# uber-research/deep-neuroevolution

Hardware: NVIDIA H100
Metric: env-steps/sec across ES population (whole box) (higher is better)
Workload: dtype f32

## Files before the change

### deep-neuroevolution_b200/csrc/common.cuh

```cuda
#pragma once
#include <cuda_runtime.h>
#include <stdint.h>
#include <stdio.h>
#include <stdarg.h>
#include <string.h>

#include "../../include/dne.h"

#if defined(__CUDA_ARCH__) && (__CUDA_ARCH__ != 900)
#error "libdne is written for sm_90a (H100) only"
#endif

#define DNE_MAX_PREP 16
struct dne_ctx {
    int device;
    int sm_count;
    const float* noise;
    int64_t noise_count;
    double* scratch;
    cudaEvent_t* ev;
    int ev_cap, ev_n, prof_on;
    void* ev_wait;
    void* ev_record;
    int ev_record_done;
    int ev_mode;
    struct { const void* ws; const float* theta; int n_slots; } prep[DNE_MAX_PREP];
};
void dne_prep_invalidate_theta(dne_ctx* ctx, const float* d_theta);
extern unsigned long long g_dne_launches;
#define DNE_LAUNCHED(n) (g_dne_launches += (unsigned long long)(n))
#define DNE_SCRATCH_DOUBLES 16384

void dne_set_error(const char* fmt, ...);

#define DNE_CHECK_ARG(cond, msg)                                   \
    do {                                                           \
        if (!(cond)) {                                             \
            dne_set_error("%s: %s", __func__, msg);                \
            return DNE_ERR_ARG;                                    \
        }                                                          \
    } while (0)

#define DNE_CUDA(call)                                                                 \
    do {                                                                               \
        cudaError_t e__ = (call);                                                      \
        if (e__ != cudaSuccess) {                                                      \
            dne_set_error("%s: %s -> %s", __func__, #call, cudaGetErrorString(e__));   \
            return DNE_ERR_CUDA;                                                       \
        }                                                                              \
    } while (0)

#define DNE_LAUNCH_CHECK1() do { DNE_LAUNCHED(1); DNE_LAUNCH_CHECK(); } while (0)
// ... 83 lines not shown
```

### deep-neuroevolution_b200/csrc/dne_api.cu

```cuda
#include "common.cuh"
#include "forward.cuh"

static thread_local char g_err[512] = "";
unsigned long long g_dne_launches = 0;
int g_dne_theta_tma = 1;
int g_dne_chain_ticks = 0;
int g_dne_pdl = 1;
int g_dne_fold_theta = 1;
int g_dne_fuse_head = 1;

void dne_set_error(const char* fmt, ...) {
    va_list ap;
    va_start(ap, fmt);
    vsnprintf(g_err, sizeof(g_err), fmt, ap);
    va_end(ap);
}

extern "C" const char* dne_last_error(void) { return g_err; }
extern "C" int dne_version(void) { return 100; }
extern "C" int dne_abi_sizes(int* layer_desc_bytes, int* net_desc_bytes) {
    if (layer_desc_bytes) *layer_desc_bytes = (int)sizeof(dne_layer_desc);
    if (net_desc_bytes) *net_desc_bytes = (int)sizeof(dne_net_desc);
    return DNE_OK;
}

extern "C" int dne_ctx_create(int device, dne_ctx** out) {
    DNE_CHECK_ARG(out, "out is null");
    *out = nullptr;
    int n = 0;
    DNE_CUDA(cudaGetDeviceCount(&n));
    DNE_CHECK_ARG(device >= 0 && device < n, "no such CUDA device");
    DNE_CUDA(cudaSetDevice(device));
    cudaDeviceProp prop;
    DNE_CUDA(cudaGetDeviceProperties(&prop, device));
    if (prop.major != 9 || prop.minor != 0) {
        dne_set_error("dne_ctx_create: device %d is sm_%d%d; libdne is built for sm_90a (H100) only", device,
                      prop.major, prop.minor);
        return DNE_ERR_CUDA;
    }
    dne_ctx* c = new dne_ctx();
    c->device = device;
    c->sm_count = prop.multiProcessorCount;
    c->noise = nullptr;
    c->noise_count = 0;
    c->scratch = nullptr;
    c->ev = nullptr;
    c->ev_cap = c->ev_n = c->prof_on = 0;
    c->ev_wait = c->ev_record = nullptr;
    c->ev_record_done = 0;
    c->ev_mode = 0;
    for (int i = 0; i < DNE_MAX_PREP; ++i) c->prep[i].ws = nullptr, c->prep[i].theta = nullptr;
    cudaError_t e = cudaMalloc(&c->scratch, sizeof(double) * DNE_SCRATCH_DOUBLES);
    if (e != cudaSuccess) {
        delete c;
        dne_set_error("dne_ctx_create: cudaMalloc -> %s", cudaGetErrorString(e));
        return DNE_ERR_CUDA;
    }
    *out = c;
    return DNE_OK;
}

extern "C" int dne_ctx_destroy(dne_ctx* ctx) {
    if (!ctx) return DNE_OK;
    cudaSetDevice(ctx->device);
    if (ctx->scratch) cudaFree(ctx->scratch);
    if (ctx->ev) {
        for (int i = 0; i < 2 * ctx->ev_cap; ++i) cudaEventDestroy(ctx->ev[i]);
        delete[] ctx->ev;
    }
    delete ctx;
    return DNE_OK;
}

extern "C" int dne_set_option(const char* name, int value) {
    DNE_CHECK_ARG(name, "name is null");
    if (strcmp(name, "conv_tc") == 0 && value >= 0 && value <= 2) { g_dne_conv_tc = value; return DNE_OK; }
    if (strcmp(name, "gemv_bulk") == 0) { g_dne_gemv_bulk = value ? 1 : 0; return DNE_OK; }
    if (strcmp(name, "fuse_head") == 0) { g_dne_fuse_head = value ? 1 : 0; return DNE_OK; }
    if (strcmp(name, "theta_mc") == 0) { extern int g_dne_theta_mc; g_dne_theta_mc = value ? 1 : 0; return DNE_OK; }
    if (strcmp(name, "theta_tma") == 0) { g_dne_theta_tma = value ? 1 : 0; return DNE_OK; }
    if (strcmp(name, "gemv_stages") == 0 && value >= 2 && value <= 8) { extern int g_dne_gemv_stages; g_dne_gemv_stages = value; return DNE_OK; }
    if (strcmp(name, "fold_theta") == 0 && value >= 0 && value <= 1) { g_dne_fold_theta = value; return DNE_OK; }
    if (strcmp(name, "chain_ticks") == 0 && value >= 0 && value <= 1) { g_dne_chain_ticks = value; return DNE_OK; }
    if (strcmp(name, "pdl") == 0 && value >= 0 && value <= 1) { g_dne_pdl = value; return DNE_OK; }
    if (strcmp(name, "gemv_grid") == 0 && value >= 0) { extern int g_dne_gemv_grid; g_dne_gemv_grid = value; return DNE_OK; }
    if (strcmp(name, "gemv_ctas_per_sm") == 0 && value >= 1 && value <= 2) { g_dne_gemv_ctas_per_sm = value; return DNE_OK; }
    dne_set_error("dne_set_option: unknown option '%s'", name);
    return DNE_ERR_ARG;
}

extern "C" long long dne_launch_count(int reset) {
    const long long v = (long long)g_dne_launches;
    if (reset) g_dne_launches = 0;
    return v;
}

extern "C" int dne_profile_enable(dne_ctx* ctx, int on, int capacity) {
    DNE_CHECK_ARG(ctx, "ctx is null");
    if (on == 2) {
        ctx->prof_on = ctx->ev ? 1 : 0;
        return DNE_OK;
    }
    if (on) {
        if (capacity < 1) capacity = 4096;
        if (capacity > ctx->ev_cap) {
            if (ctx->ev) {
                for (int i = 0; i < 2 * ctx->ev_cap; ++i) cudaEventDestroy(ctx->ev[i]);
                delete[] ctx->ev;
            }
            ctx->ev = new cudaEvent_t[2 * (size_t)capacity];
            for (int i = 0; i < 2 * capacity; ++i) DNE_CUDA(cudaEventCreate(&ctx->ev[i]));
            ctx->ev_cap = capacity;
        }
        ctx->ev_n = 0;
    }
    ctx->prof_on = on ? 1 : 0;
    return DNE_OK;
}

extern "C" int dne_profile_read(dne_ctx* ctx, int* n_launches, double* total_ms) {
    DNE_CHECK_ARG(ctx && n_launches && total_ms, "bad arguments");
    DNE_CUDA(cudaDeviceSynchronize());
    double tot = 0.0;
    for (int i = 0; i < ctx->ev_n; ++i) {
        float ms = 0.f;
        DNE_CUDA(cudaEventElapsedTime(&ms, ctx->ev[2 * i], ctx->ev[2 * i + 1]));
        tot += ms;
    }
    *n_launches = ctx->ev_n;
    *total_ms = tot;
    return DNE_OK;
}

extern "C" int dne_noise_bind(dne_ctx* ctx, const float* d_noise, int64_t count) {
    DNE_CHECK_ARG(ctx && d_noise && count > 0, "bad arguments");
    DNE_CHECK_ARG(((uintptr_t)d_noise & 15) == 0, "noise table must be 16-byte aligned");
    ctx->noise = d_noise;
    ctx->noise_count = count;
    return DNE_OK;
}

constexpr int PLAN_SM_COUNT = 132;

struct ForwardPlan {
    size_t x0_off;
    size_t act_off[DNE_MAX_LAYERS];
    int64_t act_elems[DNE_MAX_LAYERS];
    DensePlan dense[DNE_MAX_LAYERS];
    size_t part_theta_off, part_noise_off;
    size_t xc_off[DNE_MAX_LAYERS], wc_off[DNE_MAX_LAYERS];
    size_t total;
};

static bool tgm_candidate(const dne_net_desc* net, int l, const DensePlan& dp) {
    if (l == 0 || net->layers[l].kind != DNE_DENSE || net->layers[l - 1].kind != DNE_CONV || !dp.decomposed) return false;
    if (!dne_s2d_supported(net->layers[l - 1], l - 1 == 0)) return false;
    return dne_tgm_supported(net->layers[l].cin, net->layers[l].cout, dp.k_per_split);
}

static int64_t layer_out_elems(const dne_layer_desc& L) {
    return L.kind == DNE_CONV ? (int64_t)L.hout * L.hout * L.cout : (int64_t)L.cout;
}

static int plan_forward(const dne_net_desc* net, int n_slots, int paired, bool shared_theta, ForwardPlan* fp) {
// ... 370 lines not shown
```

### deep-neuroevolution_b200/csrc/forward.cuh

```cuda
#pragma once
#include "common.cuh"

struct SlotArgs {
    const float* theta;
    const float* noise;
    const int64_t* noise_idx;
    const float* scale;
    const int32_t* theta_idx;
    const uint8_t* active;
    int64_t P;
};

struct LayerEpi {
    int64_t off_b, off_beta, off_gamma;
    int act, bn, bn_off, vbn_len;
    const float* vbn;
};

struct GemvSrc {
    const float* base;
    const int64_t* idx64;
    const int32_t* idx32;
    int64_t mul, off;
};

extern int g_dne_gemv_bulk;
extern int g_dne_fold_theta;
extern int g_dne_gemv_ctas_per_sm;
int dne_launch_member_gemm_tc(const SlotArgs& sa, int64_t off_w, int64_t off_b, const float* X, int64_t x_slot_stride, int M,
                              int K, int N, float* out, int64_t out_slot_stride, int n_slots, cudaStream_t st);
constexpr int DNE_GEMV_BLOCK_ROWS = 256;
int dne_gemv_pieces(int K);
int dne_launch_gemv_union(const SlotArgs& sa, const GemvSrc& src, int G, const float* X, int64_t x_slot_stride, int K,
                          int N, int n_pieces, int n_slots, float* part, int sm_count, cudaStream_t st,
                          const float* fold_theta = nullptr, int fold_n_split = 0);

struct DensePlan {
    bool decomposed;
    int n_split, k_per_split;
    int G, Gt, rows_per_chunk, n_chunks, rw;
    size_t part_theta_floats, part_noise_floats;
};

extern int g_dne_conv_tc;
int dne_launch_conv_layer_tc(const SlotArgs& sa, const dne_layer_desc& L, const LayerEpi& epi, bool in_u8,
                             const void* in, int64_t in_slot_stride, int64_t in_img_stride, float* out,
                             int64_t out_slot_stride, int64_t out_img_stride, int n_slots, int n_img,
                             cudaStream_t st);
int dne_launch_conv_layer_simt(const SlotArgs& sa, const dne_layer_desc& L, const LayerEpi& epi, bool in_u8,
                               const void* in, int64_t in_slot_stride, int64_t in_img_stride, float* out,
                               int64_t out_slot_stride, int64_t out_img_stride, int n_slots, int n_img,
                               cudaStream_t st);

DensePlan dne_plan_dense(const dne_layer_desc& L, int n_slots, int paired, bool shared_theta, int sm_count);

int dne_launch_conv_layer(const SlotArgs& sa, const dne_layer_desc& L, const LayerEpi& epi, bool in_u8,
                          const void* in, int64_t in_slot_stride, int64_t in_img_stride, float* out,
                          int64_t out_slot_stride, int64_t out_img_stride, int n_slots, int n_img,
                          cudaStream_t st);

struct DenseHead {
    const dne_layer_desc* L;
    LayerEpi epi;
    float* out;
    int64_t out_slot_stride;
    int32_t* actions;
};
bool dne_head_fusable(const dne_layer_desc& L, const DensePlan& p, const dne_layer_desc& head, const DensePlan& hp);
// ... 41 lines not shown
```

### deep-neuroevolution_b200/csrc/forward_kernels.cu

```cuda
#include "common.cuh"
#include "forward.cuh"
#include "epilogue.cuh"

constexpr int CONV_BK = 16;

template <int CIN, int COUT, int KS, int STRIDE, int HIN, int HOUT, int PAD, bool IN_U8, int BM, int TM, int TN>
__global__ void __launch_bounds__((BM / TM) * (COUT / TN))
conv_kernel(SlotArgs sa, int64_t off_w, LayerEpi epi, const void* __restrict__ in_base, int64_t in_slot_stride,
            int64_t in_img_stride, float* __restrict__ out_base, int64_t out_slot_stride, int64_t out_img_stride) {
    constexpr int THREADS = (BM / TM) * (COUT / TN);
    constexpr int M = HOUT * HOUT;
    constexpr int K = KS * KS * CIN;
    constexpr int BK = CONV_BK;
    static_assert(K % BK == 0 && CIN % 4 == 0 && TM % 4 == 0, "tile constraints");
    constexpr int A_UNITS = BM * BK / 4;
    constexpr int A_PER_THREAD = (A_UNITS + THREADS - 1) / THREADS;
    constexpr int B_ELEMS = BK * COUT;
    constexpr int B_PER_THREAD = (B_ELEMS + THREADS - 1) / THREADS;

    const int slot = blockIdx.y;
    if (!slot_active(sa, slot)) return;
    const int img = blockIdx.z;
    const int m_tile = blockIdx.x * BM;
    const int tid = threadIdx.x;
// ... 591 lines not shown
}

int dne_launch_dense_layer(const dne_ctx* ctx, const SlotArgs& sa, const dne_layer_desc& L, const LayerEpi& epi,
                           const DensePlan& p, const float* X, int64_t x_slot_stride, float* out,
                           int64_t out_slot_stride, int32_t* actions, float* part_theta, float* part_noise,
                           int n_slots, cudaStream_t st, const DenseHead* head, const TgmOperands* tgm) {
    const int K = L.cin, N = L.cout;
    if (!p.decomposed) {
        if (actions && N > DS_MAXN) return DNE_ERR_UNSUP;
        dense_small_kernel<<<dim3(n_slots, (N + DS_MAXN - 1) / DS_MAXN), DS_THREADS, 0, st>>>(
            sa, L.off_w, epi, X, x_slot_stride, K, N, out, out_slot_stride, actions);
        DNE_LAUNCHED(1);
        return 0;
    }
    if (x_slot_stride != K || actions) return DNE_ERR_UNSUP;
    const int threads = (N / 4) * p.rw;
    auto gemv_smem = [&](int G) {
        size_t sm1 = (size_t)G * (p.rows_per_chunk + 1) * sizeof(float);
        size_t sm2 = (size_t)p.rw * G * (N + 4) * sizeof(float);
        return sm1 > sm2 ? sm1 : sm2;
    };
    if (p.Gt == 0) {
        if (tgm && dne_launch_theta_gemm_tma(tgm->Xc, tgm->Wc, n_slots, K, N, p.k_per_split, p.n_split, part_theta, st) == 0) {
        } else if (!(g_dne_conv_tc && dne_launch_theta_gemm_tc(X, n_slots, K, N, sa.theta + L.off_w, p.k_per_split, p.n_split,
                                                        part_theta, st) == 0)) {
            dim3 grid((N + DG_BN - 1) / DG_BN, (n_slots + DG_BM - 1) / DG_BM, p.n_split);
            dense_theta_gemm_kernel<<<grid, DG_THREADS, 0, st>>>(X, n_slots, K, N, sa.theta + L.off_w, p.k_per_split,
                                                                part_theta);
        }
    } else {
        GemvSrc ts{sa.theta, nullptr, sa.theta_idx, sa.P, L.off_w};
        dim3 grid(p.n_chunks, (n_slots + p.Gt - 1) / p.Gt);
        if (g_dne_gemv_bulk && dne_launch_gemv_union(sa, ts, p.Gt, X, x_slot_stride, K, N, p.n_chunks, n_slots, part_theta,
                                                     ctx->sm_count, st) == 0) {
        } else if (p.Gt == 2)
            dense_noise_gemv_kernel<2, 8><<<grid, threads, gemv_smem(2), st>>>(sa, ts, X, x_slot_stride, K, N,
                                                                              p.rows_per_chunk, part_theta);
        else
            dense_noise_gemv_kernel<1, 8><<<grid, threads, gemv_smem(1), st>>>(sa, ts, X, x_slot_stride, K, N,
                                                                              p.rows_per_chunk, part_theta);
    }
    bool folded = false;
    {
        GemvSrc ns{sa.noise, sa.noise_idx, nullptr, 0, L.off_w};
        dne_ctx* mctx = const_cast<dne_ctx*>(ctx);
        const bool first_gemv = !ctx->ev_record_done;
        if (first_gemv && ctx->ev_mode == 0 && ctx->ev_record) {
            cudaEventRecord((cudaEvent_t)ctx->ev_record, st);
            mctx->ev_record_done = 1;
        }
        if (first_gemv && ctx->ev_mode == 1 && ctx->ev_wait) {
            cudaStreamWaitEvent(st, (cudaEvent_t)ctx->ev_wait, 0);
            mctx->ev_wait = nullptr;
        }
        const int groups = (n_slots + p.G - 1) / p.G;
        dim3 grid(p.n_chunks, groups);
        const bool prof = ctx->prof_on && ctx->ev_n < ctx->ev_cap;
        if (prof) cudaEventRecord(ctx->ev[2 * ctx->ev_n], st);
        folded = g_dne_gemv_bulk && g_dne_fold_theta && p.Gt == 0;
        if (g_dne_gemv_bulk && dne_launch_gemv_union(sa, ns, p.G, X, x_slot_stride, K, N, p.n_chunks, n_slots, part_noise,
                                                     ctx->sm_count, st, folded ? part_theta : nullptr,
                                                     folded ? p.n_split : 0) == 0) {
        } else if ((folded = false), p.G == 2)
            dense_noise_gemv_kernel<2, 8><<<grid, threads, gemv_smem(2), st>>>(sa, ns, X, x_slot_stride, K, N,
                                                                              p.rows_per_chunk, part_noise);
        else
            dense_noise_gemv_kernel<1, 8><<<grid, threads, gemv_smem(1), st>>>(sa, ns, X, x_slot_stride, K, N,
                                                                              p.rows_per_chunk, part_noise);
        if (prof) {
            cudaEventRecord(ctx->ev[2 * ctx->ev_n + 1], st);
            const_cast<dne_ctx*>(ctx)->ev_n++;
        }
        if (first_gemv && ctx->ev_mode == 1 && ctx->ev_record) {
            cudaEventRecord((cudaEvent_t)ctx->ev_record, st);
            mctx->ev_record_done = 1;
        }
    }
    if (head) {
        if (dne_launch_chain(dense_combine_head_kernel, dim3(n_slots), dim3(DCH_THREADS), 0, st, true, sa, epi, n_slots, N, p.G,
                             (const float*)part_theta, folded ? -1 : p.n_split, p.Gt, (const float*)part_noise, p.n_chunks, out, out_slot_stride,
                             (int64_t)head->L->off_w, head->epi, (int)head->L->cout, head->out, head->out_slot_stride,
                             head->actions) != cudaSuccess)
            return DNE_ERR_CUDA;
    } else {
        dim3 grid((N + 255) / 256, n_slots);
        dense_combine_kernel<<<grid, 256, 0, st>>>(sa, epi, n_slots, N, p.G, part_theta, folded ? -1 : p.n_split, p.Gt, part_noise,
                                                  p.n_chunks, out, out_slot_stride);
    }
    DNE_LAUNCHED(3);
    return 0;
}

void dne_launch_ob_norm(const float* obs, const float* mean, const float* stdv, int64_t total, int dim, float* out,
                        cudaStream_t st) {
// ... 4 lines not shown
```

### deep-neuroevolution_b200/csrc/gemv_bulk.cu

```cuda
#include <climits>
#include "common.cuh"
#include "forward.cuh"
#include "epilogue.cuh"
#include "wgmma.cuh"

using namespace wg;

int g_dne_gemv_bulk = 1;
int g_dne_gemv_ctas_per_sm = 2;
int g_dne_gemv_grid = 0;
int g_dne_gemv_stages = 5;

constexpr int GB_CONSUMERS = 256;
constexpr int GB_THREADS = GB_CONSUMERS + 32;
constexpr int GB_STAGES = 8;
constexpr int GB_STAGE_BYTES = 16384;
constexpr int GB_RPR = 4;
constexpr int GU_BLK = DNE_GEMV_BLOCK_ROWS;
constexpr int GU_VEC = 8;
constexpr int GU_VB = 4;
constexpr int GU_MIN_N = 64;
constexpr int GU_XS_LD_MAX = GU_BLK + 4096 / GU_MIN_N;
constexpr int GU_XS_FLOATS = GU_VEC * GU_XS_LD_MAX > (1024 / GU_MIN_N) * GU_VB * (GU_MIN_N + 4)
                                 ? GU_VEC * GU_XS_LD_MAX : (1024 / GU_MIN_N) * GU_VB * (GU_MIN_N + 4);
constexpr int GU_PLAN_BYTES_PER_GROUP = 8 + 5 * 4;

__device__ __forceinline__ int gu_cover(const int* pb0, const int* pb1, int n_groups, int b, int first, int cap, int* out,
                                        int lane) {
    int total = 0;
    for (int h0 = 0; h0 < n_groups; h0 += 32) {
        const int h = h0 + lane;
        const bool c = h < n_groups && pb0[h] <= b && b <= pb1[h];
        const unsigned m = __ballot_sync(0xffffffffu, c);
        const int ord = total + __popc(m & ((1u << lane) - 1u));
        if (c && ord >= first && ord < first + cap) out[ord - first] = h;
        total += __popc(m);
    }
    __syncwarp();
    return total;
}

template <int G>
__global__ void __launch_bounds__(GB_THREADS, 2)
gemv_union_kernel(SlotArgs sa, GemvSrc src, const float* __restrict__ X, int64_t x_slot_stride, int K, int N,
                  int n_pieces, int n_groups, int n_slots, float* __restrict__ part, int n_stages,
                  const float* __restrict__ tpart, int t_split) {
    constexpr int CAP = GU_VEC / G;
    extern __shared__ uint8_t smem_raw[];
    uint8_t* smem = (uint8_t*)(((uintptr_t)smem_raw + 127) & ~(uintptr_t)127);
    float* stage_base = reinterpret_cast<float*>(smem);
    int64_t* pE0 = reinterpret_cast<int64_t*>(smem + n_stages * GB_STAGE_BYTES);
    int* pb0 = reinterpret_cast<int*>(pE0 + n_groups);
    int* pb1 = pb0 + n_groups;
    int* psort = pb1 + n_groups;
    int* pstart = psort + n_groups;
    int* ppre = pstart + n_groups;
    __shared__ uint64_t full_bar[GB_STAGES], empty_bar[GB_STAGES];
    __shared__ __align__(16) float xs[GU_XS_FLOATS];
    __shared__ int cov_c[CAP], cov_p[CAP];
    __shared__ int rho_c[CAP];
    __shared__ int s_total, s_row0, s_nelem, s_items;

    const int tid = threadIdx.x, warp = tid >> 5, lane = tid & 31;
    const int NQ = N >> 2;
    const int RW = GB_CONSUMERS / NQ;
    const int RB = GB_RPR * RW;
    const int XS_LD = GU_BLK + RB;
    pdl_trigger();

    if (tid == 0) {
        for (int s = 0; s < n_stages; ++s) {
            mbar_init(&full_bar[s], 1);
            mbar_init(&empty_bar[s], GB_CONSUMERS / 32);
        }
        fence_mbar_init();
    }
    for (int g = tid; g < n_groups; g += GB_THREADS) {
        const int slot0 = g * G;
        bool any = false;
#pragma unroll
        for (int m = 0; m < G; ++m) any = any || (slot0 + m < n_slots && slot_active(sa, slot0 + m));
        const int64_t E0 = (src.idx64 ? src.idx64[slot0] : (src.idx32 ? (int64_t)src.idx32[slot0] * src.mul : 0)) + src.off;
        pE0[g] = E0;
        pb0[g] = any ? (int)(E0 / N / GU_BLK) : INT_MAX;
        pb1[g] = any ? (int)((E0 + (int64_t)K * N - 1) / N / GU_BLK) : -1;
    }
    __syncthreads();
    for (int g = tid; g < n_groups; g += GB_THREADS) {
        const int key = pb0[g];
        int r = 0;
        for (int h = 0; h < n_groups; ++h) {
            const int kh = pb0[h];
            r += (kh < key) || (kh == key && h < g);
        }
        psort[r] = g;
    }
    __syncthreads();
    if (warp == 0) {
        int carry_max = -1, carry_sum = 0;
        for (int i0 = 0; i0 < n_groups; i0 += 32) {
            const int i = i0 + lane;
            const int g = i < n_groups ? psort[i] : 0;
            const int b0 = i < n_groups ? pb0[g] : INT_MAX, b1 = i < n_groups ? pb1[g] : -1;
            int mx = b1;
#pragma unroll
            for (int d = 1; d < 32; d <<= 1) {
                const int o = __shfl_up_sync(0xffffffffu, mx, d);
                if (lane >= d) mx = max(mx, o);
            }
            int before = __shfl_up_sync(0xffffffffu, mx, 1);
            if (lane == 0) before = -1;
            before = max(before, carry_max);
            const int start = max(b0, before + 1);
            const int add = (b0 != INT_MAX && b1 >= start) ? b1 - start + 1 : 0;
            int sum = add;
#pragma unroll
            for (int d = 1; d < 32; d <<= 1) {
                const int o = __shfl_up_sync(0xffffffffu, sum, d);
                if (lane >= d) sum += o;
            }
            if (i < n_groups) { pstart[i] = start; ppre[i] = carry_sum + sum - add; }
            carry_sum += __shfl_sync(0xffffffffu, sum, 31);
            carry_max = max(carry_max, __shfl_sync(0xffffffffu, mx, 31));
        }
        if (lane == 0) s_items = carry_sum;
    }
    __syncthreads();
    const int n_items = s_items;
    auto item_block = [&](int q) {
        int lo = 0, hi = n_groups;
        while (lo < hi) {
            const int mid = (lo + hi) >> 1;
            if (ppre[mid] <= q) lo = mid + 1; else hi = mid;
        }
        return pstart[lo - 1] + (q - ppre[lo - 1]);
    };
    auto pass_range = [&](int b, const int* gl, int ng, int64_t& row0, int& n_elem) {
        int64_t r_first = INT64_MAX, e_last = 0;
        for (int i = 0; i < ng; ++i) {
            const int64_t E0 = pE0[gl[i]];
            r_first = min(r_first, E0 / N);
            e_last = max(e_last, (E0 + (int64_t)K * N + 3) & ~(int64_t)3);
        }
        const int64_t blk0 = (int64_t)b * GU_BLK;
        row0 = max(r_first, blk0);
        const int64_t e_end = min(e_last, (blk0 + GU_BLK) * N);
        n_elem = (int)(e_end - row0 * N);
    };

    if (warp == GB_CONSUMERS / 32) {
        uint32_t it = 0;
        for (int item = blockIdx.x; item < n_items; item += gridDim.x) {
            const int b = item_block(item);
            int total = CAP;
            for (int first = 0; first < total; first += CAP) {
                total = gu_cover(pb0, pb1, n_groups, b, first, CAP, cov_p, lane);
                int64_t row0;
                int n_elem;
                pass_range(b, cov_p, min(CAP, total - first), row0, n_elem);
                const float* gsrc = src.base + row0 * N;
                for (int e0 = 0; e0 < n_elem; e0 += RB * N, ++it) {
                    if (lane == 0) {
                        const int s = it % n_stages;
                        mbar_wait(&empty_bar[s], ((it / n_stages) & 1) ^ 1);
                        const uint32_t bytes = (uint32_t)min(RB * N, n_elem - e0) * 4;
                        mbar_arrive_expect_tx(&full_bar[s], bytes);
                        bulk_g2s(stage_base + (size_t)s * (GB_STAGE_BYTES / 4), gsrc + e0, bytes, &full_bar[s]);
                    }
                }
                __syncwarp();
            }
        }
        return;
    }

    pdl_wait();
    const int t = tid % NQ, rw = tid / NQ;
    const int red_ld = N + 4;
    float* red = xs;
    uint32_t it = 0;
    for (int item = blockIdx.x; item < n_items; item += gridDim.x) {
        const int b = item_block(item);
        int total = CAP;
        for (int first = 0; first < total; first += CAP) {
            if (warp == 0) {
                const int tot = gu_cover(pb0, pb1, n_groups, b, first, CAP, cov_c, lane);
                if (lane == 0) {
                    const int ng = min(CAP, tot - first);
                    int64_t row0;
                    int n_elem;
                    pass_range(b, cov_c, ng, row0, n_elem);
                    s_total = tot;
                    s_row0 = (int)(row0 - (int64_t)b * GU_BLK);
                    s_nelem = n_elem;
                    for (int i = 0; i < ng; ++i) rho_c[i] = (int)(pE0[cov_c[i]] % N);
                }
            }
            named_bar_sync(1, GB_CONSUMERS);
            total = s_total;
            const int ng = min(CAP, total - first), nv = ng * G;
            const int lrow0 = s_row0, n_elem = s_nelem;
            for (int i = tid; i < nv * XS_LD; i += GB_CONSUMERS) {
                const int v = i / XS_LD, L = i - v * XS_LD - 1;
                const int g = cov_c[v / G], slot = g * G + v % G;
                const int64_t k = (int64_t)b * GU_BLK + L - pE0[g] / N;
                xs[v * XS_LD + L + 1] = (k >= 0 && k < K && slot < n_slots) ? X[(int64_t)slot * x_slot_stride + k] : 0.0f;
            }
            named_bar_sync(1, GB_CONSUMERS);

            float acc[GU_VEC][4];
#pragma unroll
            for (int v = 0; v < GU_VEC; ++v)
#pragma unroll
                for (int c = 0; c < 4; ++c) acc[v][c] = 0.0f;

            for (int e0 = 0; e0 < n_elem; e0 += RB * N, ++it) {
                const int s = it % n_stages;
                const int stage_elems = min(RB * N, n_elem - e0);
                const int rl0 = rw * GB_RPR;
                const int xb0 = lrow0 + e0 / N + rl0;
                mbar_wait(&full_bar[s], (it / n_stages) & 1);
                const uint32_t rows_a = wg::smem_u32(stage_base) + s * GB_STAGE_BYTES + (rl0 * NQ + t) * 16;
                float4 w[GB_RPR];
#pragma unroll
                for (int j = 0; j < GB_RPR; ++j)
                    w[j] = ((rl0 + j) * N + 4 * t < stage_elems) ? wg::lds128(rows_a + j * NQ * 16) : make_float4(0.f, 0.f, 0.f, 0.f);
#pragma unroll
                for (int gi = 0; gi < CAP; ++gi) {
                    if (gi < ng) {
                        const int rho = rho_c[gi];
                        const bool p0 = 4 * t < rho, p1 = 4 * t + 1 < rho, p2 = 4 * t + 2 < rho, p3 = 4 * t + 3 < rho;
#pragma unroll
                        for (int m = 0; m < G; ++m) {
                            const int v = gi * G + m;
                            float xm[GB_RPR + 1];
#pragma unroll
                            for (int j = 0; j <= GB_RPR; ++j) xm[j] = xs[v * XS_LD + xb0 + j];
#pragma unroll
                            for (int j = 0; j < GB_RPR; ++j) {
                                acc[v][0] = fmaf(p0 ? xm[j] : xm[j + 1], w[j].x, acc[v][0]);
                                acc[v][1] = fmaf(p1 ? xm[j] : xm[j + 1], w[j].y, acc[v][1]);
                                acc[v][2] = fmaf(p2 ? xm[j] : xm[j + 1], w[j].z, acc[v][2]);
                                acc[v][3] = fmaf(p3 ? xm[j] : xm[j + 1], w[j].w, acc[v][3]);
                            }
                        }
                    }
                }
                __syncwarp();
                if (lane == 0) mbar_arrive(&empty_bar[s]);
            }
            for (int vb0 = 0; vb0 < nv; vb0 += GU_VB) {
                named_bar_sync(1, GB_CONSUMERS);
#pragma unroll
                for (int v = 0; v < GU_VEC; ++v) {
                    if (v >= vb0 && v < vb0 + GU_VB && v < nv) {
                        const int rho = rho_c[v / G];
                        float* row = red + (rw * GU_VB + (v - vb0)) * red_ld;
#pragma unroll
                        for (int c = 0; c < 4; ++c) {
                            const int n = 4 * t + c - rho;
                            row[n < 0 ? n + N : n] = acc[v][c];
                        }
                    }
                }
                named_bar_sync(1, GB_CONSUMERS);
                for (int i = tid; i < GU_VB * N; i += GB_CONSUMERS) {
                    const int vl = i / N, n = i - vl * N, v = vb0 + vl;
                    if (v >= nv) break;
                    const int g = cov_c[v / G], m = v % G, slot = g * G + m;
                    const int piece = b - pb0[g];
                    float sum = 0.0f;
                    for (int w2 = 0; w2 < RW; ++w2) sum += red[(w2 * GU_VB + vl) * red_ld + n];
                    if (tpart) {
                        float ts = 0.0f;
                        if (slot < n_slots)
                            for (int j = piece; j < t_split; j += n_pieces) ts += tpart[((int64_t)j * n_slots + slot) * N + n];
                        sum = fmaf(slot < n_slots ? sa.scale[slot] : 0.0f, sum, ts);
                    }
                    part[(((int64_t)g * n_pieces + piece) * G + m) * N + n] = sum;
                }
            }
            for (int gi = 0; gi < ng; ++gi) {
                const int g = cov_c[gi];
                if (pb1[g] != b) continue;
                for (int piece = b - pb0[g] + 1; piece < n_pieces; ++piece)
                    for (int i = tid; i < G * N; i += GB_CONSUMERS) {
                        const int m = i / N, n = i - m * N, slot = g * G + m;
                        float ts = 0.0f;
                        if (tpart && slot < n_slots)
                            for (int j = piece; j < t_split; j += n_pieces) ts += tpart[((int64_t)j * n_slots + slot) * N + n];
                        part[(((int64_t)g * n_pieces + piece) * G + m) * N + n] = ts;
                    }
            }
            named_bar_sync(1, GB_CONSUMERS);
        }
    }
}

int dne_gemv_pieces(int K) { return (K + 1 + GU_BLK - 1) / GU_BLK + 1; }

int dne_launch_gemv_union(const SlotArgs& sa, const GemvSrc& src, int G, const float* X, int64_t x_slot_stride, int K,
                          int N, int n_pieces, int n_slots, float* part, int sm_count, cudaStream_t st,
                          const float* fold_theta, int fold_n_split) {
    if (N % 4 != 0 || N < GU_MIN_N || N * 4 > GB_STAGE_BYTES || (GB_CONSUMERS % (N / 4)) != 0) return DNE_ERR_UNSUP;
    const int RW = GB_CONSUMERS / (N / 4);
    if (GB_RPR * RW * N * 4 != GB_STAGE_BYTES || n_pieces != dne_gemv_pieces(K) || (G != 1 && G != 2)) return DNE_ERR_UNSUP;
    const int n_groups = (n_slots + G - 1) / G;
    if (n_groups <= 0) return 0;
    const size_t static_smem = (size_t)GU_XS_FLOATS * 4 + 1024;
    const size_t plan = (size_t)n_groups * GU_PLAN_BYTES_PER_GROUP + 128;
    const size_t per_sm = 227 * 1024;
    int cps = g_dne_gemv_ctas_per_sm, n_stages = 0;
    for (; cps >= 1; --cps) {
        const size_t budget = per_sm / cps - 1024;
        n_stages = budget > static_smem + plan ? (int)((budget - static_smem - plan) / GB_STAGE_BYTES) : 0;
        if (n_stages > g_dne_gemv_stages) n_stages = g_dne_gemv_stages;
        if (n_stages >= 2) break;
    }
    if (cps < 1) return DNE_ERR_UNSUP;
    const size_t smem = (size_t)n_stages * GB_STAGE_BYTES + plan;
    int grid = cps * sm_count;
    if (g_dne_gemv_grid > 0 && grid > g_dne_gemv_grid) grid = g_dne_gemv_grid;
    int dev = 0;
    cudaGetDevice(&dev);
    static bool attr_done_dev[64][3] = {};
    bool* attr_done = attr_done_dev[dev < 64 ? dev : 63];
    auto launch = [&](auto kern) -> int {
        if (!attr_done[G]) {
            cudaFuncSetAttribute(kern, cudaFuncAttributePreferredSharedMemoryCarveout, cudaSharedmemCarveoutMaxShared);
            if (cudaFuncSetAttribute(kern, cudaFuncAttributeMaxDynamicSharedMemorySize, (int)(per_sm - static_smem - 1024)) != cudaSuccess)
                return DNE_ERR_CUDA;
            attr_done[G] = true;
        }
        if (dne_launch_chain(kern, dim3(grid), dim3(GB_THREADS), smem, st, true, sa, src, X, x_slot_stride, K, N, n_pieces,
                             n_groups, n_slots, part, n_stages, fold_theta, fold_theta ? fold_n_split : 0) != cudaSuccess)
            return DNE_ERR_CUDA;
        return 0;
    };
    return G == 2 ? launch(gemv_union_kernel<2>) : launch(gemv_union_kernel<1>);
}
```

### deep-neuroevolution_b200/dne/_ffi.py

```python
from __future__ import annotations

import ctypes as C
import os
from typing import Optional

import torch

_HERE = os.path.dirname(os.path.abspath(__file__))
LIB_PATH = os.environ.get("DNE_LIB") or os.path.join(_HERE, "libdne.so")

DNE_MAX_LAYERS = 8
CONV, DENSE = 0, 1
ACT_NONE, ACT_RELU, ACT_TANH = 0, 1, 2
BN_NONE, BN_TF, BN_GPU = 0, 1, 2
OB_ATARI_U8, OB_VECTOR = 0, 1
EPISODE_CARTPOLE, EPISODE_ACROBOT, EPISODE_MOUNTAINCAR = 0, 1, 2


class LayerDesc(C.Structure):
    _fields_ = [("kind", C.c_int32), ("cin", C.c_int32), ("cout", C.c_int32), ("ksize", C.c_int32),
                ("stride", C.c_int32), ("hin", C.c_int32), ("hout", C.c_int32), ("pad", C.c_int32),
                ("act", C.c_int32), ("bn", C.c_int32), ("bn_off", C.c_int32), ("_pad", C.c_int32),
                ("off_w", C.c_int64), ("off_b", C.c_int64), ("off_beta", C.c_int64), ("off_gamma", C.c_int64)]

# ... 15 lines not shown
    "dne_ctx_create": [C.c_int, C.POINTER(_P)],
    "dne_ctx_destroy": [_P],
    "dne_noise_bind": [_P, _P, C.c_int64],
    "dne_forward_ws_bytes": [C.POINTER(NetDesc), C.c_int, C.POINTER(C.c_size_t)],
    "dne_perturb_forward_conv": [_P, C.POINTER(NetDesc), _P, _P, _P, _P, _P, C.c_int, C.c_int, _P, _P, _P, _P, _P,
                                 C.c_size_t, _P],
    "dne_perturb_forward_mlp": [_P, C.POINTER(NetDesc), _P, _P, _P, _P, _P, C.c_int, C.c_int, _P, _P, _P, _P, _P,
                                C.c_size_t, _P],
    "dne_ob_stat_accumulate": [_P, C.c_int, _P, C.c_int, _P, _P, _P],
    "dne_cartpole_episodes": [_P, C.POINTER(NetDesc), _P, _P, _P, _P, C.c_int, _P, C.c_int, _P, _P, _P, _P],
    "dne_discrete_episodes": [_P, C.c_int, C.POINTER(NetDesc), _P, _P, _P, _P, C.c_int, _P, C.c_int, _P, _P, _P, _P],
    "dne_pendulum_net_supported": [C.POINTER(NetDesc)],
    "dne_pendulum_episodes": [_P, C.POINTER(NetDesc), _P, _P, _P, _P, C.c_int, _P, C.c_int, _P, _P, _P, _P, _P, _P, _P,
                              _P, _P, _P],
    "dne_theta_prepare": [_P, C.POINTER(NetDesc), _P, C.c_int, _P, C.c_size_t, _P],
    "dne_theta_forget": [_P, _P],
    "dne_vbn_ws_bytes": [C.POINTER(NetDesc), C.c_int, C.c_int, C.POINTER(C.c_size_t)],
    "dne_vbn_reference_pass": [_P, C.POINTER(NetDesc), _P, _P, _P, _P, _P, C.c_int, _P, C.c_int, _P, _P,
                               C.c_size_t, _P],
    "dne_preprocess_atari": [_P, _P, _P, _P, C.c_int, C.c_int, _P],
    "dne_warp_atari_rgb": [_P, _P, C.c_int, _P],
    "dne_warp_atari_palette": [_P, _P, _P, _P, C.c_int, _P],
    "dne_centered_rank": [_P, C.c_int, _P, _P, _P],
    "dne_es_grad": [_P, _P, _P, C.c_int, C.c_int64, C.c_double, _P, C.c_int, _P],
    "dne_adam_step": [_P, _P, _P, _P, _P, C.c_int64, C.c_double, C.c_double, C.c_double, C.c_double, C.c_double,
                      C.c_int, _P, _P],
    "dne_sgd_step": [_P, _P, _P, _P, C.c_int64, C.c_double, C.c_double, C.c_double, _P, _P],
    "dne_ga_materialize": [_P, C.POINTER(NetDesc), _P, _P, C.c_int, C.POINTER(C.c_double), C.c_int, _P, _P],
    "dne_abi_sizes": [C.POINTER(C.c_int), C.POINTER(C.c_int)],
    "dne_set_option": [C.c_char_p, C.c_int],
    "dne_set_phase_events": [_P, _P, _P, C.c_int],
    "dne_profile_enable": [_P, C.c_int, C.c_int],
    "dne_profile_read": [_P, C.POINTER(C.c_int), C.POINTER(C.c_double)],
    "dne_ga_mutate": [_P, _P, C.c_int64, C.c_float, C.c_int64, _P, _P],
    "dne_ga_truncate": [_P, C.c_int, C.c_int, _P, _P],
    "dne_knn_ws_bytes": [C.c_int, C.c_int, C.POINTER(C.c_size_t)],
    "dne_knn_novelty_vec": [_P, C.c_int, _P, C.c_int, C.c_int, C.c_int, _P, _P, C.c_size_t, _P],
    "dne_knn_novelty": [_P, _P, C.c_int, _P, _P, C.c_int, C.c_int, C.c_int, C.c_int, _P, _P, C.c_size_t, _P],
}
EXPORTS = sorted(list(_SIGS) + ["dne_last_error", "dne_version", "dne_launch_count"])


def lib():
    global _lib
    if _lib is None:
        if not os.path.exists(LIB_PATH):
            raise DneError(f"{LIB_PATH} not built: run `python -c 'import __graft_entry__ as g; g.build()'` "
                           "(there is no CPU fallback)")
        L = C.CDLL(LIB_PATH)
        for name, args in _SIGS.items():
            fn = getattr(L, name)
            fn.argtypes = args
            fn.restype = C.c_int
        L.dne_last_error.restype = C.c_char_p
        L.dne_last_error.argtypes = []
        L.dne_version.restype = C.c_int
        L.dne_version.argtypes = []
        L.dne_launch_count.restype = C.c_longlong
        L.dne_launch_count.argtypes = [C.c_int]
        a, b = C.c_int(), C.c_int()
        L.dne_abi_sizes(C.byref(a), C.byref(b))
        if (a.value, b.value) != (C.sizeof(LayerDesc), C.sizeof(NetDesc)):
            raise DneError(f"ABI mismatch: C structs {a.value}/{b.value} bytes, ctypes {C.sizeof(LayerDesc)}/{C.sizeof(NetDesc)}")
        _lib = L
    return _lib

# ... 70 lines not shown
```

### include/dne.h

```cpp
#ifndef DNE_H_
#define DNE_H_

#include <stddef.h>
#include <stdint.h>

#ifdef __cplusplus
extern "C" {
#endif

#define DNE_OK            0
#define DNE_ERR_ARG      -1
#define DNE_ERR_CUDA     -2
#define DNE_ERR_WS       -3
#define DNE_ERR_UNSUP    -4

#define DNE_MAX_LAYERS    8

#define DNE_CONV   0
#define DNE_DENSE  1
#define DNE_ACT_NONE 0
#define DNE_ACT_RELU 1
#define DNE_ACT_TANH 2
#define DNE_BN_NONE 0
#define DNE_BN_TF   1
// ... 8 lines not shown
    int32_t ksize, stride;
    int32_t hin, hout, pad;
    int32_t act;
    int32_t bn;
    int32_t bn_off;
    int32_t _pad;
    int64_t off_w, off_b;
    int64_t off_beta, off_gamma;
} dne_layer_desc;

typedef struct dne_net_desc {
    int32_t n_layers;
    int32_t ob_kind;
    int32_t ob_dim;
    int32_t n_out;
    int32_t vbn_len;
    int32_t _pad;
    int64_t num_params;
    dne_layer_desc layers[DNE_MAX_LAYERS];
} dne_net_desc;

typedef struct dne_ctx dne_ctx;

int         dne_ctx_create(int device, dne_ctx** out);
int         dne_ctx_destroy(dne_ctx* ctx);
const char* dne_last_error(void);
int         dne_version(void);
int         dne_abi_sizes(int* layer_desc_bytes, int* net_desc_bytes);

long long   dne_launch_count(int reset);
int         dne_set_option(const char* name, int value);
int         dne_profile_enable(dne_ctx* ctx, int on, int capacity);
int         dne_profile_read(dne_ctx* ctx, int* n_launches, double* total_ms);

int dne_noise_bind(dne_ctx* ctx, const float* d_noise, int64_t count);

int dne_forward_ws_bytes(const dne_net_desc* net, int n_slots, size_t* out_bytes);

int dne_perturb_forward_conv(dne_ctx* ctx, const dne_net_desc* net, const float* d_theta,
                             const int64_t* d_noise_idx, const float* d_scale, const int32_t* d_theta_idx,
                             const uint8_t* d_active, int n_slots, int paired,
                             const uint8_t* d_obs, const float* d_vbn,
                             int32_t* d_actions, float* d_logits,
                             void* d_ws, size_t ws_bytes, void* stream);

int dne_theta_prepare(dne_ctx* ctx, const dne_net_desc* net, const float* d_theta, int n_slots, void* d_ws, size_t ws_bytes,
                      void* stream);
int dne_theta_forget(dne_ctx* ctx, const void* d_ws);

int dne_set_phase_events(dne_ctx* ctx, void* wait_event, void* record_event, int mode);

int dne_perturb_forward_mlp(dne_ctx* ctx, const dne_net_desc* net, const float* d_theta,
                            const int64_t* d_noise_idx, const float* d_scale, const int32_t* d_theta_idx,
                            const uint8_t* d_active, int n_slots, int paired,
                            const float* d_obs, const float* d_ob_mean, const float* d_ob_std,
                            float* d_actions_out, void* d_ws, size_t ws_bytes, void* stream);

int dne_cartpole_episodes(dne_ctx* ctx, const dne_net_desc* net, const float* d_theta,
                          const int64_t* d_noise_idx, const float* d_scale, const int32_t* d_theta_idx,
                          int n_members, const double* d_init_state, int max_steps,
                          float* d_returns, int32_t* d_lengths, double* d_final_state, void* stream);

#define DNE_EPISODE_CARTPOLE    0
#define DNE_EPISODE_ACROBOT     1
#define DNE_EPISODE_MOUNTAINCAR 2

// ... 59 lines not shown
```

Before: 345,000.

## Schedule gemv union work items dynamically via atomic counter queue and add tracing

```diff
diff --git a/deep-neuroevolution_b200/csrc/common.cuh b/deep-neuroevolution_b200/csrc/common.cuh
--- a/deep-neuroevolution_b200/csrc/common.cuh
+++ b/deep-neuroevolution_b200/csrc/common.cuh
@@ -12,12 +12,14 @@
 #endif
 
 #define DNE_MAX_PREP 16
+#define DNE_GEMV_CTR_SLOTS 64
 struct dne_ctx {
     int device;
     int sm_count;
     const float* noise;
     int64_t noise_count;
     double* scratch;
+    unsigned* gemv_ctr;
     cudaEvent_t* ev;
     int ev_cap, ev_n, prof_on;
     void* ev_wait;
diff --git a/deep-neuroevolution_b200/csrc/dne_api.cu b/deep-neuroevolution_b200/csrc/dne_api.cu
--- a/deep-neuroevolution_b200/csrc/dne_api.cu
+++ b/deep-neuroevolution_b200/csrc/dne_api.cu
@@ -44,6 +44,7 @@
     c->noise = nullptr;
     c->noise_count = 0;
     c->scratch = nullptr;
+    c->gemv_ctr = nullptr;
     c->ev = nullptr;
     c->ev_cap = c->ev_n = c->prof_on = 0;
     c->ev_wait = c->ev_record = nullptr;
@@ -51,7 +52,11 @@
     c->ev_mode = 0;
     for (int i = 0; i < DNE_MAX_PREP; ++i) c->prep[i].ws = nullptr, c->prep[i].theta = nullptr;
     cudaError_t e = cudaMalloc(&c->scratch, sizeof(double) * DNE_SCRATCH_DOUBLES);
+    if (e == cudaSuccess) e = cudaMalloc(&c->gemv_ctr, sizeof(unsigned) * 2 * DNE_GEMV_CTR_SLOTS);
+    if (e == cudaSuccess) e = cudaMemset(c->gemv_ctr, 0, sizeof(unsigned) * 2 * DNE_GEMV_CTR_SLOTS);
     if (e != cudaSuccess) {
+        if (c->scratch) cudaFree(c->scratch);
+        if (c->gemv_ctr) cudaFree(c->gemv_ctr);
         delete c;
         dne_set_error("dne_ctx_create: cudaMalloc -> %s", cudaGetErrorString(e));
         return DNE_ERR_CUDA;
@@ -64,6 +69,7 @@
     if (!ctx) return DNE_OK;
     cudaSetDevice(ctx->device);
     if (ctx->scratch) cudaFree(ctx->scratch);
+    if (ctx->gemv_ctr) cudaFree(ctx->gemv_ctr);
     if (ctx->ev) {
         for (int i = 0; i < 2 * ctx->ev_cap; ++i) cudaEventDestroy(ctx->ev[i]);
         delete[] ctx->ev;
@@ -85,6 +91,7 @@
     if (strcmp(name, "pdl") == 0 && value >= 0 && value <= 1) { g_dne_pdl = value; return DNE_OK; }
     if (strcmp(name, "gemv_grid") == 0 && value >= 0) { extern int g_dne_gemv_grid; g_dne_gemv_grid = value; return DNE_OK; }
     if (strcmp(name, "gemv_ctas_per_sm") == 0 && value >= 1 && value <= 2) { g_dne_gemv_ctas_per_sm = value; return DNE_OK; }
+    if (strcmp(name, "gemv_trace") == 0 && value >= 0) { extern int g_dne_gemv_trace; g_dne_gemv_trace = value; return DNE_OK; }
     dne_set_error("dne_set_option: unknown option '%s'", name);
     return DNE_ERR_ARG;
 }
@@ -130,6 +137,14 @@
     *n_launches = ctx->ev_n;
     *total_ms = tot;
     return DNE_OK;
+}
+
+extern "C" int dne_gemv_trace_read(unsigned long long* host, long long cap_words, int* grid, int* passes_per_cta) {
+    DNE_CHECK_ARG(host && grid && passes_per_cta, "bad arguments");
+    const int rc = dne_gemv_trace_copy(host, cap_words, grid, passes_per_cta);
+    if (rc == DNE_ERR_ARG) dne_set_error("dne_gemv_trace_read: buffer too small");
+    if (rc == DNE_ERR_CUDA) dne_set_error("dne_gemv_trace_read: %s", cudaGetErrorString(cudaGetLastError()));
+    return rc;
 }
 
 extern "C" int dne_noise_bind(dne_ctx* ctx, const float* d_noise, int64_t count) {
diff --git a/deep-neuroevolution_b200/csrc/forward.cuh b/deep-neuroevolution_b200/csrc/forward.cuh
--- a/deep-neuroevolution_b200/csrc/forward.cuh
+++ b/deep-neuroevolution_b200/csrc/forward.cuh
@@ -32,8 +32,9 @@
 constexpr int DNE_GEMV_BLOCK_ROWS = 256;
 int dne_gemv_pieces(int K);
 int dne_launch_gemv_union(const SlotArgs& sa, const GemvSrc& src, int G, const float* X, int64_t x_slot_stride, int K,
-                          int N, int n_pieces, int n_slots, float* part, int sm_count, cudaStream_t st,
+                          int N, int n_pieces, int n_slots, float* part, int sm_count, unsigned* ctr, cudaStream_t st,
                           const float* fold_theta = nullptr, int fold_n_split = 0);
+int dne_gemv_trace_copy(unsigned long long* host, long long cap_words, int* grid, int* passes_per_cta);
 
 struct DensePlan {
     bool decomposed;
diff --git a/deep-neuroevolution_b200/csrc/forward_kernels.cu b/deep-neuroevolution_b200/csrc/forward_kernels.cu
--- a/deep-neuroevolution_b200/csrc/forward_kernels.cu
+++ b/deep-neuroevolution_b200/csrc/forward_kernels.cu
@@ -647,7 +647,7 @@
         GemvSrc ts{sa.theta, nullptr, sa.theta_idx, sa.P, L.off_w};
         dim3 grid(p.n_chunks, (n_slots + p.Gt - 1) / p.Gt);
         if (g_dne_gemv_bulk && dne_launch_gemv_union(sa, ts, p.Gt, X, x_slot_stride, K, N, p.n_chunks, n_slots, part_theta,
-                                                     ctx->sm_count, st) == 0) {
+                                                     ctx->sm_count, ctx->gemv_ctr, st) == 0) {
         } else if (p.Gt == 2)
             dense_noise_gemv_kernel<2, 8><<<grid, threads, gemv_smem(2), st>>>(sa, ts, X, x_slot_stride, K, N,
                                                                               p.rows_per_chunk, part_theta);
@@ -674,7 +674,7 @@
         if (prof) cudaEventRecord(ctx->ev[2 * ctx->ev_n], st);
         folded = g_dne_gemv_bulk && g_dne_fold_theta && p.Gt == 0;
         if (g_dne_gemv_bulk && dne_launch_gemv_union(sa, ns, p.G, X, x_slot_stride, K, N, p.n_chunks, n_slots, part_noise,
-                                                     ctx->sm_count, st, folded ? part_theta : nullptr,
+                                                     ctx->sm_count, ctx->gemv_ctr, st, folded ? part_theta : nullptr,
                                                      folded ? p.n_split : 0) == 0) {
         } else if ((folded = false), p.G == 2)
             dense_noise_gemv_kernel<2, 8><<<grid, threads, gemv_smem(2), st>>>(sa, ns, X, x_slot_stride, K, N,
diff --git a/deep-neuroevolution_b200/csrc/gemv_bulk.cu b/deep-neuroevolution_b200/csrc/gemv_bulk.cu
--- a/deep-neuroevolution_b200/csrc/gemv_bulk.cu
+++ b/deep-neuroevolution_b200/csrc/gemv_bulk.cu
@@ -1,3 +1,4 @@
+#include <atomic>
 #include <climits>
 #include "common.cuh"
 #include "forward.cuh"
@@ -10,6 +11,10 @@
 int g_dne_gemv_ctas_per_sm = 2;
 int g_dne_gemv_grid = 0;
 int g_dne_gemv_stages = 5;
+int g_dne_gemv_trace = 0;
+static unsigned long long* g_trace_buf = nullptr;
+static size_t g_trace_words = 0;
+static int g_trace_grid = 0, g_trace_cap = 0;
 
 constexpr int GB_CONSUMERS = 256;
 constexpr int GB_THREADS = GB_CONSUMERS + 32;
@@ -23,7 +28,15 @@
 constexpr int GU_XS_LD_MAX = GU_BLK + 4096 / GU_MIN_N;
 constexpr int GU_XS_FLOATS = GU_VEC * GU_XS_LD_MAX > (1024 / GU_MIN_N) * GU_VB * (GU_MIN_N + 4)
                                  ? GU_VEC * GU_XS_LD_MAX : (1024 / GU_MIN_N) * GU_VB * (GU_MIN_N + 4);
-constexpr int GU_PLAN_BYTES_PER_GROUP = 8 + 5 * 4;
+constexpr int GU_PLAN_BYTES_PER_GROUP = 2 * 8 + 6 * 4;
+constexpr int GU_TR_HDR = 8, GU_TR_PASS = 6;
+constexpr int GU_QUEUE = 2 * GB_STAGES;
+
+__device__ __forceinline__ unsigned long long gu_globaltimer() {
+    unsigned long long t;
+    asm volatile("mov.u64 %0, %%globaltimer;" : "=l"(t));
+    return t;
+}
 
 __device__ __forceinline__ int gu_cover(const int* pb0, const int* pb1, int n_groups, int b, int first, int cap, int* out,
                                         int lane) {
@@ -44,13 +57,16 @@
 __global__ void __launch_bounds__(GB_THREADS, 2)
 gemv_union_kernel(SlotArgs sa, GemvSrc src, const float* __restrict__ X, int64_t x_slot_stride, int K, int N,
                   int n_pieces, int n_groups, int n_slots, float* __restrict__ part, int n_stages,
-                  const float* __restrict__ tpart, int t_split) {
+                  const float* __restrict__ tpart, int t_split, unsigned* ctr, unsigned long long* __restrict__ trace,
+                  int trace_cap) {
     constexpr int CAP = GU_VEC / G;
     extern __shared__ uint8_t smem_raw[];
     uint8_t* smem = (uint8_t*)(((uintptr_t)smem_raw + 127) & ~(uintptr_t)127);
     float* stage_base = reinterpret_cast<float*>(smem);
     int64_t* pE0 = reinterpret_cast<int64_t*>(smem + n_stages * GB_STAGE_BYTES);
-    int* pb0 = reinterpret_cast<int*>(pE0 + n_groups);
+    int64_t* pR = pE0 + n_groups;
+    int* prho = reinterpret_cast<int*>(pR + n_groups);
+    int* pb0 = prho + n_groups;
     int* pb1 = pb0 + n_groups;
     int* psort = pb1 + n_groups;
     int* pstart = psort + n_groups;
@@ -58,8 +74,10 @@
     __shared__ uint64_t full_bar[GB_STAGES], empty_bar[GB_STAGES];
     __shared__ __align__(16) float xs[GU_XS_FLOATS];
     __shared__ int cov_c[CAP], cov_p[CAP];
-    __shared__ int rho_c[CAP];
+    __shared__ int rho_c[CAP], kb_c[CAP];
     __shared__ int s_total, s_row0, s_nelem, s_items;
+    __shared__ uint64_t item_bar[GU_QUEUE];
+    __shared__ int q_item[GU_QUEUE];
 
     const int tid = threadIdx.x, warp = tid >> 5, lane = tid & 31;
     const int NQ = N >> 2;
@@ -67,12 +85,15 @@
     const int RB = GB_RPR * RW;
     const int XS_LD = GU_BLK + RB;
     pdl_trigger();
+    unsigned long long* tr = trace ? trace + (size_t)blockIdx.x * (GU_TR_HDR + GU_TR_PASS * trace_cap) : nullptr;
+    if (tr && tid == 0) { tr[0] = gu_globaltimer(); tr[1] = clock64(); }
 
     if (tid == 0) {
         for (int s = 0; s < n_stages; ++s) {
             mbar_init(&full_bar[s], 1);
             mbar_init(&empty_bar[s], GB_CONSUMERS / 32);
         }
+        for (int q = 0; q < GU_QUEUE; ++q) mbar_init(&item_bar[q], 1);
         fence_mbar_init();
     }
     for (int g = tid; g < n_groups; g += GB_THREADS) {
@@ -82,6 +103,8 @@
         for (int m = 0; m < G; ++m) any = any || (slot0 + m < n_slots && slot_active(sa, slot0 + m));
         const int64_t E0 = (src.idx64 ? src.idx64[slot0] : (src.idx32 ? (int64_t)src.idx32[slot0] * src.mul : 0)) + src.off;
         pE0[g] = E0;
+        pR[g] = E0 / N;
+        prho[g] = (int)(E0 % N);
         pb0[g] = any ? (int)(E0 / N / GU_BLK) : INT_MAX;
         pb1[g] = any ? (int)((E0 + (int64_t)K * N - 1) / N / GU_BLK) : -1;
     }
@@ -138,9 +161,8 @@
     auto pass_range = [&](int b, const int* gl, int ng, int64_t& row0, int& n_elem) {
         int64_t r_first = INT64_MAX, e_last = 0;
         for (int i = 0; i < ng; ++i) {
-            const int64_t E0 = pE0[gl[i]];
-            r_first = min(r_first, E0 / N);
-            e_last = max(e_last, (E0 + (int64_t)K * N + 3) & ~(int64_t)3);
+            r_first = min(r_first, pR[gl[i]]);
+            e_last = max(e_last, (pE0[gl[i]] + (int64_t)K * N + 3) & ~(int64_t)3);
         }
         const int64_t blk0 = (int64_t)b * GU_BLK;
         row0 = max(r_first, blk0);
@@ -150,7 +172,14 @@
 
     if (warp == GB_CONSUMERS / 32) {
         uint32_t it = 0;
-        for (int item = blockIdx.x; item < n_items; item += gridDim.x) {
+        int item = blockIdx.x;
+        for (uint32_t qi = 0;; ++qi) {
+            if (item >= n_items) item = -1;
+            if (lane == 0) {
+                q_item[qi % GU_QUEUE] = item;
+                mbar_arrive(&item_bar[qi % GU_QUEUE]);
+            }
+            if (item < 0) break;
             const int b = item_block(item);
             int total = CAP;
             for (int first = 0; first < total; first += CAP) {
@@ -170,16 +199,35 @@
                 }
                 __syncwarp();
             }
+            if (qi == 0) pdl_wait();
+            int next = 0;
+            if (lane == 0) next = (int)gridDim.x + (int)atomicAdd(&ctr[0], 1u);
+            item = __shfl_sync(0xffffffffu, next, 0);
+        }
+        if (lane == 0) {
+            pdl_wait();
+            __threadfence();
+            if (atomicAdd(&ctr[1], 1u) == gridDim.x - 1) {
+                ctr[0] = 0;
+                ctr[1] = 0;
+            }
         }
         return;
     }
 
     pdl_wait();
+    const bool rec = tr && tid == 0;
+    if (rec) tr[2] = clock64();
+    int n_pass = 0;
+    unsigned long long* trp = nullptr;
     const int t = tid % NQ, rw = tid / NQ;
     const int red_ld = N + 4;
     float* red = xs;
-    uint32_t it = 0;
-    for (int item = blockIdx.x; item < n_items; item += gridDim.x) {
+    uint32_t it = 0, it0 = 0;
+    for (uint32_t qi = 0;; ++qi) {
+        mbar_wait(&item_bar[qi % GU_QUEUE], (qi / GU_QUEUE) & 1);
+        const int item = q_item[qi % GU_QUEUE];
+        if (item < 0) break;
         const int b = item_block(item);
         int total = CAP;
         for (int first = 0; first < total; first += CAP) {
@@ -193,20 +241,42 @@
                     s_total = tot;
                     s_row0 = (int)(row0 - (int64_t)b * GU_BLK);
                     s_nelem = n_elem;
-                    for (int i = 0; i < ng; ++i) rho_c[i] = (int)(pE0[cov_c[i]] % N);
+                    for (int i = 0; i < ng; ++i) {
+                        rho_c[i] = prho[cov_c[i]];
+                        kb_c[i] = (int)((int64_t)b * GU_BLK - pR[cov_c[i]]);
+                    }
                 }
             }
             named_bar_sync(1, GB_CONSUMERS);
             total = s_total;
             const int ng = min(CAP, total - first), nv = ng * G;
             const int lrow0 = s_row0, n_elem = s_nelem;
-            for (int i = tid; i < nv * XS_LD; i += GB_CONSUMERS) {
-                const int v = i / XS_LD, L = i - v * XS_LD - 1;
-                const int g = cov_c[v / G], slot = g * G + v % G;
-                const int64_t k = (int64_t)b * GU_BLK + L - pE0[g] / N;
-                xs[v * XS_LD + L + 1] = (k >= 0 && k < K && slot < n_slots) ? X[(int64_t)slot * x_slot_stride + k] : 0.0f;
+            trp = rec && n_pass < trace_cap ? tr + GU_TR_HDR + GU_TR_PASS * n_pass : nullptr;
+            ++n_pass;
+            it0 = it;
+            if (trp) trp[0] = clock64();
+            {
+                constexpr int XS_PER_T = (GU_VEC * GU_XS_LD_MAX + GB_CONSUMERS - 1) / GB_CONSUMERS;
+                float xv[XS_PER_T];
+#pragma unroll
+                for (int r = 0; r < XS_PER_T; ++r) {
+                    const int i = tid + r * GB_CONSUMERS;
+                    xv[r] = 0.0f;
+                    if (i < nv * XS_LD) {
+                        const int v = i / XS_LD, L = i - v * XS_LD - 1;
+                        const int gi = v / G, slot = cov_c[gi] * G + v % G;
+                        const int k = kb_c[gi] + L;
+                        if (k >= 0 && k < K && slot < n_slots) xv[r] = X[(int64_t)slot * x_slot_stride + k];
+                    }
+                }
+#pragma unroll
+                for (int r = 0; r < XS_PER_T; ++r) {
+                    const int i = tid + r * GB_CONSUMERS;
+                    if (i < nv * XS_LD) xs[i] = xv[r];
+                }
             }
             named_bar_sync(1, GB_CONSUMERS);
+            if (trp) trp[1] = clock64();
 
             float acc[GU_VEC][4];
 #pragma unroll
@@ -220,6 +290,7 @@
                 const int rl0 = rw * GB_RPR;
                 const int xb0 = lrow0 + e0 / N + rl0;
                 mbar_wait(&full_bar[s], (it / n_stages) & 1);
+                if (trp && it == it0) trp[2] = clock64();
                 const uint32_t rows_a = wg::smem_u32(stage_base) + s * GB_STAGE_BYTES + (rl0 * NQ + t) * 16;
                 float4 w[GB_RPR];
 #pragma unroll
@@ -249,6 +320,7 @@
                 __syncwarp();
                 if (lane == 0) mbar_arrive(&empty_bar[s]);
             }
+            if (trp) trp[3] = clock64();
             for (int vb0 = 0; vb0 < nv; vb0 += GU_VB) {
                 named_bar_sync(1, GB_CONSUMERS);
 #pragma unroll
@@ -293,14 +365,24 @@
                     }
             }
             named_bar_sync(1, GB_CONSUMERS);
-        }
+            if (trp) {
+                trp[4] = clock64();
+                trp[5] = ((unsigned long long)b << 32) | ((unsigned long long)nv << 16) | (it - it0);
+            }
+        }
+    }
+    if (rec) {
+        tr[3] = clock64();
+        tr[4] = gu_globaltimer();
+        tr[5] = n_pass;
+        tr[6] = it;
     }
 }
 
 int dne_gemv_pieces(int K) { return (K + 1 + GU_BLK - 1) / GU_BLK + 1; }
 
 int dne_launch_gemv_union(const SlotArgs& sa, const GemvSrc& src, int G, const float* X, int64_t x_slot_stride, int K,
-                          int N, int n_pieces, int n_slots, float* part, int sm_count, cudaStream_t st,
+                          int N, int n_pieces, int n_slots, float* part, int sm_count, unsigned* ctr, cudaStream_t st,
                           const float* fold_theta, int fold_n_split) {
     if (N % 4 != 0 || N < GU_MIN_N || N * 4 > GB_STAGE_BYTES || (GB_CONSUMERS % (N / 4)) != 0) return DNE_ERR_UNSUP;
     const int RW = GB_CONSUMERS / (N / 4);
@@ -321,6 +403,22 @@
     const size_t smem = (size_t)n_stages * GB_STAGE_BYTES + plan;
     int grid = cps * sm_count;
     if (g_dne_gemv_grid > 0 && grid > g_dne_gemv_grid) grid = g_dne_gemv_grid;
+    static std::atomic<unsigned> launches{0};
+    const unsigned slot = launches.fetch_add(1) % DNE_GEMV_CTR_SLOTS;
+    unsigned long long* trace = nullptr;
+    if (g_dne_gemv_trace > 0) {
+        const size_t words = (size_t)grid * (GU_TR_HDR + GU_TR_PASS * g_dne_gemv_trace);
+        if (words > g_trace_words) {
+            if (g_trace_buf) cudaFree(g_trace_buf);
+            g_trace_words = 0;
+            if (cudaMalloc(&g_trace_buf, words * 8) != cudaSuccess) return DNE_ERR_CUDA;
+            g_trace_words = words;
+        }
+        if (cudaMemsetAsync(g_trace_buf, 0, words * 8, st) != cudaSuccess) return DNE_ERR_CUDA;
+        trace = g_trace_buf;
+        g_trace_grid = grid;
+        g_trace_cap = g_dne_gemv_trace;
+    }
     int dev = 0;
     cudaGetDevice(&dev);
     static bool attr_done_dev[64][3] = {};
@@ -333,9 +431,20 @@
             attr_done[G] = true;
         }
         if (dne_launch_chain(kern, dim3(grid), dim3(GB_THREADS), smem, st, true, sa, src, X, x_slot_stride, K, N, n_pieces,
-                             n_groups, n_slots, part, n_stages, fold_theta, fold_theta ? fold_n_split : 0) != cudaSuccess)
+                             n_groups, n_slots, part, n_stages, fold_theta, fold_theta ? fold_n_split : 0, ctr + 2 * slot, trace,
+                             g_dne_gemv_trace) != cudaSuccess)
             return DNE_ERR_CUDA;
         return 0;
     };
     return G == 2 ? launch(gemv_union_kernel<2>) : launch(gemv_union_kernel<1>);
 }
+
+int dne_gemv_trace_copy(unsigned long long* host, long long cap_words, int* grid, int* passes_per_cta) {
+    *grid = g_trace_grid;
+    *passes_per_cta = g_trace_cap;
+    const size_t words = (size_t)g_trace_grid * (GU_TR_HDR + GU_TR_PASS * g_trace_cap);
+    if (!g_trace_buf || words == 0) return 0;
+    if ((long long)words > cap_words) return DNE_ERR_ARG;
+    if (cudaDeviceSynchronize() != cudaSuccess) return DNE_ERR_CUDA;
+    return cudaMemcpy(host, g_trace_buf, words * 8, cudaMemcpyDeviceToHost) == cudaSuccess ? 0 : DNE_ERR_CUDA;
+}
diff --git a/deep-neuroevolution_b200/dne/_ffi.py b/deep-neuroevolution_b200/dne/_ffi.py
--- a/deep-neuroevolution_b200/dne/_ffi.py
+++ b/deep-neuroevolution_b200/dne/_ffi.py
@@ -71,6 +71,7 @@
     "dne_set_phase_events": [_P, _P, _P, C.c_int],
     "dne_profile_enable": [_P, C.c_int, C.c_int],
     "dne_profile_read": [_P, C.POINTER(C.c_int), C.POINTER(C.c_double)],
+    "dne_gemv_trace_read": [_P, C.c_longlong, C.POINTER(C.c_int), C.POINTER(C.c_int)],
     "dne_ga_mutate": [_P, _P, C.c_int64, C.c_float, C.c_int64, _P, _P],
     "dne_ga_truncate": [_P, C.c_int, C.c_int, _P, _P],
     "dne_knn_ws_bytes": [C.c_int, C.c_int, C.POINTER(C.c_size_t)],
diff --git a/include/dne.h b/include/dne.h
--- a/include/dne.h
+++ b/include/dne.h
@@ -64,6 +64,7 @@
 int         dne_set_option(const char* name, int value);
 int         dne_profile_enable(dne_ctx* ctx, int on, int capacity);
 int         dne_profile_read(dne_ctx* ctx, int* n_launches, double* total_ms);
+int         dne_gemv_trace_read(unsigned long long* host, long long cap_words, int* grid, int* passes_per_cta);
 
 int dne_noise_bind(dne_ctx* ctx, const float* d_noise, int64_t count);
 
```

After: 387,300 (median of 6 runs). 1.12x the previous value.
